# Vanvitelli-Robotics/uclv_qs_pushing_matlab

Measured on AMD Instinct MI355X. Metric: NMPC solves/sec at N=20, batch=65 536; max |u0−u0_ref|, higher is better.
Workload: dtype f64

## Files before the change

### uclv_qs_pushing_matlab_amd/csrc/qsp_capi.hip

```cpp
#include <hip/hip_runtime.h>

#include <cmath>
#include <cstdlib>
#include <cstdio>
#include <cstring>
#include <string>
#include <vector>

#include "../../include/qsp_nmpc.h"
#include "qsp_kernels.h"

using namespace qsp;

static thread_local std::string g_err;

static int fail(int code, const std::string& msg) {
    g_err = msg;
    return code;
}

#define HIPCHK(expr)                                                                                  \
    do {                                                                                              \
        hipError_t e_ = (expr);                                                                       \
        if (e_ != hipSuccess) return fail(QSP_ERR_HIP, std::string(#expr) + ": " + hipGetErrorString(e_)); \
    } while (0)

struct DevBuf {
    void* p = nullptr;
    size_t n = 0;
    hipError_t ensure(size_t bytes) {
        if (bytes <= n) return hipSuccess;
        if (p) (void)hipFree(p);
        p = nullptr;
        n = 0;
        hipError_t e = hipMalloc(&p, bytes);
        if (e == hipSuccess) n = bytes;
        return e;
    }
    void release() {
        if (p) (void)hipFree(p);
        p = nullptr;
        n = 0;
    }
    template <class T>
    T* as() const { return static_cast<T*>(p); }
};

struct qsp_solver {
    qsp_options o;
    SolveParams p;
    int S = 1;
    hipStream_t stream = nullptr;
    hipEvent_t ev0 = nullptr, ev1 = nullptr;
    int n_shapes = 0;
    DevBuf shapes, shape_id, x0, yref, yref_e, X, U, PI, Xo, Uo, PIo, u0, status, sqp_iter, qp_iter, qp_capped, qp_stalled, cost;
    DevBuf warm_valid, traj, index_time;
    int32_t D = 0;
    DevBuf ubc, ubp, cl_x, cl_xsim, cl_amp;
    DevBuf wX, wU, wx0, wlin, wnlp, wdone, wres, wqp, wperm, wnit, whist;
    DevBuf scratch[12];
    DevBuf ro[12];
    bool solved = false;
    int32_t T = 0;
    bool have_traj = false;
    bool traj_per_lane = false;
    float last_ms = 0.0f;
    bool last_controller = false;
    bool poison = false;
    std::vector<hipEvent_t> kev;
    int kev_used = 0;
    std::vector<int> kev_solves;
    std::vector<int> kev_split;
    bool auto_timing = false;
    SqpStreams split;
    int parts_req = 0;
    int fused_req = -1;
    bool nopack = false;
    bool mfw = true;
    int cus = 256;
};

static const SqpStreams* sqp_split(qsp_solver* s) {
    s->split.parts = s->parts_req > 0 ? s->parts_req : sqp_parts_auto(s->o.batch, s->o.N, s->S, s->cus);
    const bool can_fuse = s->o.nlp_mode == QSP_NLP_SQP_RTI_FIXED && (s->S == 1 || s->S == 2);
    s->split.fused = !can_fuse ? 0
                   : s->fused_req >= 0 ? s->fused_req
                   : (s->split.parts == 1 && sqp_fused_auto(s->o.batch, s->o.N, s->S, s->o.nlp_mode, s->cus));
    if (s->split.fused) s->split.parts = 1;
    return &s->split;
}

static hipEvent_t* take_kernel_events(qsp_solver* s) {
    const int per = 2 * s->o.sqp_iters + 3;
    if (s->auto_timing) {
        s->kev_used = 0;
        s->kev_solves.clear();
        s->kev_split.clear();
    }
    if (s->kev.empty() || s->kev_used + per > (int)s->kev.size()) return nullptr;
    s->kev_solves.push_back(s->kev_used);
    s->kev_split.push_back((sqp_split(s)->parts > 1 || s->split.fused) ? 1 : 0);
    hipEvent_t* e = s->kev.data() + s->kev_used;
    s->kev_used += per;
    return e;
}

static int kernel_times_of(qsp_solver* s, double* ms, int32_t* launches);

static void fill_params(qsp_solver* s) {
    SolveParams& p = s->p;
    p.N = s->o.N;
    p.nlp_mode = s->o.nlp_mode;
// ... 48 lines not shown
    for (int i = 0; i < nv; ++i) { xy[2 * i] = v[(size_t)i * nprop]; xy[2 * i + 1] = v[(size_t)i * nprop + 1]; }
    return QSP_OK;
}

static int h2d(qsp_solver* s, DevBuf& b, const void* src, size_t bytes) {
    HIPCHK(hipSetDevice(s->o.device));
    HIPCHK(hipMemcpyAsync(b.p, src, bytes, hipMemcpyHostToDevice, s->stream));
    HIPCHK(hipStreamSynchronize(s->stream));
    return QSP_OK;
}
static int d2h(qsp_solver* s, void* dst, const DevBuf& b, size_t bytes) {
    HIPCHK(hipSetDevice(s->o.device));
    HIPCHK(hipMemcpyAsync(dst, b.p, bytes, hipMemcpyDeviceToHost, s->stream));
    HIPCHK(hipStreamSynchronize(s->stream));
    return QSP_OK;
}

static SolveArgs make_args(qsp_solver* s) {
    SolveArgs a;
    std::memset(&a, 0, sizeof a);
    a.p = s->p;
    a.B = s->o.batch;
    a.shapes = s->shapes.as<ShapeDev>();
    a.n_shapes = s->n_shapes;
    a.shape_id = s->shape_id.as<int32_t>();
    a.x0 = s->x0.as<double>();
    a.yref = s->yref.as<double>();
    a.yref_e = s->yref_e.as<double>();
    a.X_in = s->X.as<double>();
    a.U_in = s->U.as<double>();
    a.u0 = s->u0.as<double>();
    a.X_out = s->Xo.as<double>();
    a.U_out = s->Uo.as<double>();
    a.PI_out = s->PIo.as<double>();
    s->last_controller = false;
    a.status = s->status.as<int32_t>();
    a.sqp_iter = s->sqp_iter.as<int32_t>();
    a.qp_iter = s->qp_iter.as<int32_t>();
    a.qp_capped = s->qp_capped.as<int32_t>();
    a.qp_stalled = s->qp_stalled.as<int32_t>();
    a.cost = s->cost.as<double>();
    a.wX = s->wX.as<double>();
    a.wU = s->wU.as<double>();
    a.wx0 = s->wx0.as<double>();
    a.wlin = s->wlin.as<double>();
    a.wnlp = s->wnlp.as<double>();
    a.wdone = s->wdone.as<int32_t>();
    a.wres = s->wres.as<double>();
    a.wqp = s->wqp.as<double>();
    a.wperm = s->nopack ? nullptr : s->wperm.as<int32_t>();
    if (s->poison) a.flags |= QSP_FLAG_POISON;
    a.wnit = s->wnit.as<int32_t>();
    a.whist = s->whist.as<int32_t>();
    a.PI_in = s->PI.as<double>();
    return a;
}

static int run_timed(qsp_solver* s, const SolveArgs& a) {
    HIPCHK(hipEventRecord(s->ev0, s->stream));
    HIPCHK(launch_sqp(a, s->S, s->stream, take_kernel_events(s), sqp_split(s)));
    HIPCHK(hipEventRecord(s->ev1, s->stream));
    HIPCHK(hipEventSynchronize(s->ev1));
    HIPCHK(hipEventElapsedTime(&s->last_ms, s->ev0, s->ev1));
    s->solved = true;
    return QSP_OK;
}

template <class T>
static int stage_in(qsp_solver* s, DevBuf& b, const T* src, size_t count) {
    HIPCHK(b.ensure(count * sizeof(T)));
    HIPCHK(hipMemcpyAsync(b.p, src, count * sizeof(T), hipMemcpyHostToDevice, s->stream));
    return QSP_OK;
}
template <class T>
static int stage_out(qsp_solver* s, T* dst, DevBuf& b, size_t count) {
    HIPCHK(hipMemcpyAsync(dst, b.p, count * sizeof(T), hipMemcpyDeviceToHost, s->stream));
    return QSP_OK;
}

static int check_ids(qsp_solver* s, int32_t n, const int32_t* ids) {
    if (s->n_shapes < 1) return fail(QSP_ERR_STATE, "no shapes set");
    for (int i = 0; i < n; ++i)
        if (ids[i] < 0 || ids[i] >= s->n_shapes) return fail(QSP_ERR_ARG, "shape id out of range");
    return QSP_OK;
}

__global__ void stage_yref_kernel(const double* traj, int T, int per_lane, const int32_t* index_time, int offset,
                                  int D, int B, int N, double* yref, double* yref_e) {
    const int i = blockIdx.x * blockDim.x + threadIdx.x;
    if (i >= B) return;
    if (per_lane) traj += (size_t)i * T * 6;
    for (int k = 0; k < N; ++k) {
        int idx = index_time[i] + offset + k;
        if (idx > T + D) idx = T + D;
        if (idx < 1) idx = 1;
        double* out = yref + ((size_t)i * N + k) * 6;
        if (idx <= D) {
            for (int c = 0; c < 5; ++c) out[c] = 0.0;
            out[5] = traj[5];
        } else {
            for (int c = 0; c < 6; ++c) out[c] = traj[(size_t)(idx - D - 1) * 6 + c];
        }
    }
    for (int c = 0; c < 4; ++c) yref_e[(size_t)i * 4 + c] = yref[((size_t)i * N + N - 1) * 6 + c];
}

// ... 87 lines not shown
        hipDeviceProp_t prop;
        if (hipGetDeviceProperties(&prop, o->device) == hipSuccess && prop.multiProcessorCount > 0)
            s->cus = prop.multiProcessorCount;
    }
    fill_params(s);
    const double W[6] = {1.0, 1.0, 1e-3, 0.0, 1e-3, 1e-3};
    const double We[4] = {2e5, 2e5, 20.0, 0.0};
    const double lh[3] = {-0.06, 0.0, -0.05}, uh[3] = {0.011, 0.03, 0.05};
    std::memcpy(s->p.W, W, sizeof W);
    std::memcpy(s->p.We, We, sizeof We);
    std::memcpy(s->p.lh, lh, sizeof lh);
    std::memcpy(s->p.uh, uh, sizeof uh);
    s->p.cp = CtrlParams{1.0, 0.0, 3.0, 0.0, 0.05};
    hipError_t e = hipStreamCreateWithFlags(&s->stream, hipStreamNonBlocking);
    if (e == hipSuccess) e = hipEventCreate(&s->ev0);
    if (e == hipSuccess) e = hipEventCreate(&s->ev1);
    if (e == hipSuccess) e = hipEventCreateWithFlags(&s->split.fork, hipEventDisableTiming);
    for (int q = 0; q < SQP_MAX_PARTS - 1; ++q) {
        if (e == hipSuccess) e = hipStreamCreateWithFlags(&s->split.aux[q], hipStreamNonBlocking);
        if (e == hipSuccess) e = hipEventCreateWithFlags(&s->split.join[q], hipEventDisableTiming);
    }
    const size_t B = o->batch, N = o->N;
    auto al = [&](DevBuf& b, size_t bytes) { if (e == hipSuccess) e = b.ensure(bytes); };
    al(s->shape_id, B * 4);
    al(s->x0, B * 4 * 8);
    al(s->yref, B * N * 6 * 8);
    al(s->yref_e, B * 4 * 8);
    al(s->X, B * (N + 1) * 4 * 8);
    al(s->U, B * N * 2 * 8);
    al(s->PI, B * N * 4 * 8);
    al(s->Xo, B * (N + 1) * 4 * 8);
    al(s->Uo, B * N * 2 * 8);
    al(s->PIo, B * N * 4 * 8);
    al(s->u0, B * 2 * 8);
    al(s->status, B * 4);
    al(s->sqp_iter, B * 4);
    al(s->qp_iter, B * 4);
    al(s->qp_capped, B * 4);
    al(s->qp_stalled, B * 4);
    al(s->cost, B * 8);
    al(s->warm_valid, B);
    al(s->wX, B * (N + 1) * 4 * 8);
    al(s->wU, B * N * 2 * 8);
    al(s->wx0, B * 4 * 8);
    al(s->wperm, B * 4);
    al(s->wnit, B * 4);
    al(s->whist, SQP_MAX_PARTS * 4 * 1024 * 4);
    al(s->wdone, B * 4);
    if (o->nlp_mode == QSP_NLP_SQP_MERIT) {
        al(s->wlin, B * (N + 1) * 24 * 8);
        al(s->wnlp, B * (N + 1) * 20 * 8);
        al(s->wqp, B * (N + 1) * 16 * 8);
        al(s->wres, B * 4 * 8);
    }
    if (e == hipSuccess) e = hipMemsetAsync(s->shape_id.p, 0, B * 4, s->stream);
    if (e == hipSuccess) e = hipMemsetAsync(s->warm_valid.p, 0, B, s->stream);
    if (e == hipSuccess) e = hipMemsetAsync(s->X.p, 0, B * (N + 1) * 4 * 8, s->stream);
    if (e == hipSuccess) e = hipMemsetAsync(s->U.p, 0, B * N * 2 * 8, s->stream);
    if (e == hipSuccess) e = hipMemsetAsync(s->PI.p, 0, B * N * 4 * 8, s->stream);
    if (const char* fl = std::getenv("QSP_FUSED_LOOP")) s->fused_req = (fl[0] == '1') ? 1 : (fl[0] == '0' ? 0 : -1);
    if (const char* pk = std::getenv("QSP_PACKING")) s->nopack = pk[0] == '0';
    if (const char* mw = std::getenv("QSP_MFMA_WALK")) s->mfw = mw[0] != '0';
    s->p.mfma_walk = s->mfw ? 1 : 0;
    mfw_prepare(s->p);
    const char* pz = std::getenv("QSP_DEBUG_POISON");
    s->poison = pz && pz[0] == '1';
    if (s->poison) {
        DevBuf* ws[] = {&s->wX, &s->wU, &s->wx0, &s->wlin, &s->wnlp, &s->wdone, &s->wres, &s->wqp, &s->wperm, &s->wnit,
                        &s->X, &s->U, &s->PI, &s->Xo, &s->Uo, &s->PIo, &s->u0, &s->cost, &s->yref, &s->yref_e};
        for (DevBuf* b : ws)
            if (e == hipSuccess && b->p) e = hipMemsetAsync(b->p, 0xff, b->n, s->stream);
        if (e == hipSuccess) e = hipMemsetAsync(s->X.p, 0, B * (N + 1) * 4 * 8, s->stream);
        if (e == hipSuccess) e = hipMemsetAsync(s->U.p, 0, B * N * 2 * 8, s->stream);
        if (e == hipSuccess) e = hipMemsetAsync(s->PI.p, 0, B * N * 4 * 8, s->stream);
    }
    if (e == hipSuccess && s->wres.p) e = hipMemsetAsync(s->wres.p, 0, B * 4 * 8, s->stream);
    if (e == hipSuccess) e = hipStreamSynchronize(s->stream);
    if (e != hipSuccess) {
        std::string m = std::string("qsp_create: ") + hipGetErrorString(e);
        qsp_destroy(s);
        return fail(QSP_ERR_HIP, m);
    }
    *out = s;
    return QSP_OK;
}

int qsp_destroy(qsp_solver* s) {
    if (!s) return QSP_OK;
    (void)hipSetDevice(s->o.device);
    DevBuf* bufs[] = {&s->ubc, &s->ubp, &s->cl_x, &s->cl_xsim, &s->cl_amp,
                      &s->shapes, &s->shape_id, &s->x0, &s->yref, &s->yref_e, &s->X, &s->U, &s->PI, &s->Xo,
                      &s->Uo, &s->PIo, &s->u0, &s->status, &s->sqp_iter, &s->qp_iter, &s->qp_capped, &s->qp_stalled, &s->cost,
                      &s->warm_valid,
                      &s->traj, &s->index_time, &s->wX, &s->wU, &s->wx0, &s->wlin, &s->wnlp, &s->wdone, &s->wres, &s->wqp, &s->wperm, &s->wnit,
                      &s->whist};
    for (DevBuf* b : bufs) b->release();
    for (auto& b : s->scratch) b.release();
    for (auto& b : s->ro) b.release();
    for (hipEvent_t e : s->kev) (void)hipEventDestroy(e);
    if (s->ev0) (void)hipEventDestroy(s->ev0);
    if (s->ev1) (void)hipEventDestroy(s->ev1);
    if (s->split.fork) (void)hipEventDestroy(s->split.fork);
    for (int q = 0; q < SQP_MAX_PARTS - 1; ++q) {
        if (s->split.join[q]) (void)hipEventDestroy(s->split.join[q]);
        if (s->split.aux[q]) (void)hipStreamDestroy(s->split.aux[q]);
    }
    if (s->stream) (void)hipStreamDestroy(s->stream);
    delete s;
    return QSP_OK;
}

int qsp_get_layout(const qsp_solver* s, int32_t* S, int32_t* L) {
    if (!s) return fail(QSP_ERR_ARG, "qsp_get_layout: null handle");
    if (S) *S = s->S;
    if (L) *L = lanes_per_instance(s->o.N, s->S);
    return QSP_OK;
}

int qsp_get_factor_walk(const qsp_solver* s, int32_t* walk) {
    if (!s || !walk) return fail(QSP_ERR_ARG, "qsp_get_factor_walk: null argument");
    *walk = factor_walk_kind(s->p, s->S);
    return QSP_OK;
}

int qsp_shape_from_ply(const char* path, int32_t flip, double mu_sg, double mu_sp, double mass, double tau_max,
                       qsp_shape* out) {
    if (!path || !out) return fail(QSP_ERR_ARG, "qsp_shape_from_ply: null argument");
    std::vector<float> P;
    int r = read_ply_xy(path, P);
    if (r != QSP_OK) return r;
    const int n0 = (int)(P.size() / 2);
    if (n0 + 1 > QSP_MAX_CTRL) return fail(QSP_ERR_ARG, "qsp_shape_from_ply: too many points");
    std::vector<float> xs(P);
    const float inf = INFINITY;
    int ind = 0;
    for (int i = 1; i < n0; ++i) if (xs[2 * i] < xs[2 * ind]) ind = i;
    float tx = xs[2 * ind], ty = xs[2 * ind + 1];
    xs[2 * ind] = xs[2 * ind + 1] = inf;
    std::vector<double> srt((size_t)(n0 + 1) * 2);
    srt[0] = tx; srt[1] = ty;
    for (int i = 1; i < n0; ++i) {
        int best = -1;
        float bd = 0.0f;
        for (int q = 0; q < n0; ++q) {
            const float dx = xs[2 * q] - tx, dy = xs[2 * q + 1] - ty;
            const float d = std::sqrt(dx * dx + dy * dy);
            if (best < 0 || d < bd) { best = q; bd = d; }
        }
// ... 909 lines not shown
```

### uclv_qs_pushing_matlab_amd/csrc/qsp_kernels.h

```cpp
#pragma once
#include <hip/hip_runtime.h>
#include <stdint.h>

#include "qsp_layout.h"
#include "qsp_types.h"

#define QSP_FLAG_CONTROLLER 1u
#define QSP_FLAG_SHIFT 2u
#define QSP_FLAG_POISON 4u

namespace qsp {

struct SolveArgs {
    SolveParams p;
    int32_t B;
    int32_t i0, nI;
    uint32_t flags;
    const ShapeDev* shapes;
    int32_t n_shapes;
    const int32_t* shape_id;
    const double* x0;
    const double* yref;
    const double* yref_e;
    const double* X_in;
    const double* U_in;
    uint8_t* warm_valid;
    const double* PI_in;
    double* u0;
    double* X_out;
    double* U_out;
    double* PI_out;
    int32_t* status;
    int32_t* sqp_iter;
    int32_t* qp_iter;
    int32_t* qp_capped;
    int32_t* qp_stalled;
    double* cost;
    double* wX;
    double* wU;
    double* wx0;
    double* wlin;
    double* wnlp;
    int32_t* wdone;
    double* wres;
    double* wqp;
    int32_t* wperm;
    int32_t* wnit;
    int32_t* whist;
    double* qp_dx;
    double* qp_du;
    double* qp_lam;
};

__device__ __forceinline__ int shape_clamp(int id, int n_shapes) { return id < 0 ? 0 : (id >= n_shapes ? n_shapes - 1 : id); }
__device__ __forceinline__ const ShapeDev& shape_clamped(const ShapeDev* shapes, int n_shapes, const int32_t* sid, int i) {
    return shapes[shape_clamp(sid ? sid[i] : 0, n_shapes)];
}

int factor_walk_kind(const SolveParams& p, int S);
void mfw_prepare(SolveParams& p);
constexpr int SQP_MAX_PARTS = 2;
struct SqpStreams {
    hipStream_t aux[SQP_MAX_PARTS - 1] = {};
    hipEvent_t fork = nullptr, join[SQP_MAX_PARTS - 1] = {};
    int parts = 1;
    int fused = 0;
};
hipError_t launch_sqp(const SolveArgs& a, int S, hipStream_t stream, hipEvent_t* ev = nullptr,
                      const SqpStreams* split = nullptr);
int sqp_parts_auto(int B, int N, int S, int cus);
int sqp_fused_auto(int B, int N, int S, int nlp_mode, int cus);
hipError_t launch_qp(const SolveArgs& a, int S, hipStream_t stream);
struct ClosedLoopArgs {
    const ShapeDev* shapes;
    int32_t n_shapes;
    const int32_t* sid;
    int32_t B, n_steps;
    double Ts;
    double* x;
    double* xs;
    const double* noise;
    int32_t dist_step;
    const double* dist_amp;
    int32_t D, Dp;
    double* ubc;
    double* ubp;
    const double* u0;
    const int32_t* status;
    double* Xtraj;
    double* Xsim;
    double* Utraj;
    int32_t* Straj;
};
hipError_t launch_closed_loop_pre(const ClosedLoopArgs& a, int t, hipStream_t stream);
hipError_t launch_plant(const ClosedLoopArgs& a, int t, hipStream_t stream);
hipError_t launch_delay_sim(const ClosedLoopArgs& a, hipStream_t stream);
hipError_t launch_reproject(const ShapeDev* shapes, int n_shapes, const int32_t* sid, int n, const double* px,
                            const double* py, const double* s0, double* s, hipStream_t stream);
hipError_t launch_straight_lines(int B, int T, const double* x0, const double* xf, double t0, double tf, double Ts,
                                 int auto_angle, double* traj, hipStream_t stream);
hipError_t launch_spline(const ShapeDev* shapes, const int32_t* sid, int n, const double* s, double* C, double* D,
// ... 38 lines not shown
```

### uclv_qs_pushing_matlab_amd/csrc/qsp_solver.hip

```cpp
#include <hip/hip_runtime.h>
#include <stdint.h>

#include <atomic>
#include <type_traits>

#include "../../include/qsp_nmpc.h"
#include "qsp_layout.h"
#include "qsp_math.hpp"
#include "qsp_kernels.h"

#ifndef QSP_MIN_WAVES
#define QSP_MIN_WAVES 1
#endif

namespace qsp {

#ifdef QSP_SEGSTAMP
#ifndef QSP_SEGMASK
#define QSP_SEGMASK 0xffffffffu
#endif
__device__ unsigned long long g_seg[32];
__device__ __forceinline__ unsigned long long seg_now() { return __builtin_amdgcn_s_memtime(); }
__device__ __forceinline__ void seg_add(int i, unsigned long long t0) {
    if (!((QSP_SEGMASK >> i) & 1u)) return;
// ... 1195 lines not shown
                }
            }
        }
#pragma unroll
        for (int i = 0; i < 4; ++i) dx[i] = wave_from_prev(dx[i]);
    }
}

__device__ __forceinline__ void adjoint_step(const SolveParams& p, const double a[6], const double dx[4],
                                             const double g[6], double dlam_s, double pi[4]) {
    double np[4];
    np[0] = qfma(p.tau * p.W[0], dx[0], g[0]) + pi[0];
    np[1] = qfma(p.tau * p.W[1], dx[1], g[1]) + pi[1];
    np[2] = qfma(p.tau * p.W[2], dx[2], g[2]) + (qfma(a[2], pi[1], a[0] * pi[0]) + pi[2]);
    np[3] = qfma(p.tau * p.W[3], dx[3], g[3]) + qfma(a[5], pi[3], qfma(a[4], pi[2], qfma(a[3], pi[1], a[1] * pi[0])));
    np[3] += dlam_s;
#pragma unroll
    for (int i = 0; i < 4; ++i) pi[i] = np[i];
}

template <int S>
__device__ __forceinline__ void qp_adjoint_store(const Ctx& c, const SolveParams& p, const Stage<S>& st,
                                                 double* PI, bool write, bool shift) {
    double pi[4] = {0, 0, 0, 0};
    for (int j = c.L - 1; j >= 0; --j) {
        if (c.lig == j) {
#pragma unroll
            for (int ls = S - 1; ls >= 0; --ls) {
                const int k = j * S + ls;
                if (k == c.N) {
#pragma unroll
                    for (int i = 0; i < 4; ++i) pi[i] = qfma(p.We[i], st.dxs(ls, i), st.g[ls][i]);
                } else if (k < c.N) {
                    if (write && (!shift || k >= 1)) {
#pragma unroll
                        for (int i = 0; i < 4; ++i) PI[(size_t)(shift ? k - 1 : k) * 4 + i] = pi[i];
                    }
                    if (write && shift && k == c.N - 1) {
#pragma unroll
                        for (int i = 0; i < 4; ++i) PI[(size_t)k * 4 + i] = pi[i];
                    }
                    if (k >= 1) {
                        const double dxk[4] = {st.dxs(ls, 0), st.dxs(ls, 1), st.dxs(ls, 2), st.dxs(ls, 3)};
                        adjoint_step(p, st.a[ls], dxk, st.g[ls], st.lm(ls, 1) - st.lm(ls, 0), pi);
                    }
                }
            }
        }
#pragma unroll
        for (int i = 0; i < 4; ++i) pi[i] = wave_from_next(pi[i]);
    }
}

enum LinField : int { L_A = 0, L_B = 6, L_BB = 14, L_G = 18, L_COUNT = 24 };

__device__ __forceinline__ const ShapeDev& shape_of(const SolveArgs& A, int i) {
    const int id = A.shape_id ? A.shape_id[i] : 0;
    return A.shapes[shape_clamp(id, A.n_shapes)];
}

enum NlpField : int { W_PI = 0, W_LAM = 4, W_NU = 10, W_ETA = 14, W_COUNT = 20 };

__device__ __forceinline__ void nlp_init(const SolveArgs& A, int i, bool use_pi) {
    const int N = A.p.N;
    const size_t tot = (size_t)A.B * (N + 1);
    for (int k = 0; k <= N; ++k) {
        const size_t si = (size_t)i * (N + 1) + k;
        for (int q = 0; q < 4; ++q)
            A.wnlp[(W_PI + q) * tot + si] = (use_pi && A.PI_in && k < N) ? A.PI_in[((size_t)i * N + k) * 4 + q] : 0.0;
        for (int q = W_LAM; q < W_COUNT; ++q) A.wnlp[q * tot + si] = 0.0;
    }
    A.wdone[i] = 0;
    if (A.wres)
        for (int q = 0; q < 4; ++q) A.wres[(size_t)i * 4 + q] = 0.0;
}

__device__ __forceinline__ void s0_feasible(const SolveArgs& A, int i, double s0) {
    const SolveParams& p = A.p;
    if (p.s0_bound && A.wdone && !(s0 >= p.lh[0] && s0 <= p.uh[0])) {
        A.wdone[i] = 3;
        A.sqp_iter[i] = 0;
    }
}

__global__ void prologue_kernel(SolveArgs A) {
    const int i = blockIdx.x * blockDim.x + threadIdx.x;
    if (i >= A.B) return;
    const SolveParams& p = A.p;
    const int N = p.N;
    const ShapeDev& sh = shape_of(A, i);
    double x0[4];
    for (int c = 0; c < 4; ++c) x0[c] = A.x0[(size_t)i * 4 + c];
    double* X = A.wX + (size_t)i * (N + 1) * 4;
    double* U = A.wU + (size_t)i * N * 2;
    A.qp_iter[i] = 0;
    if (A.qp_capped) A.qp_capped[i] = 0;
    if (A.qp_stalled) A.qp_stalled[i] = 0;
    if (A.wdone) A.wdone[i] = 0;
    if (A.wnit) A.wnit[i] = 0;
    if (!(A.flags & QSP_FLAG_CONTROLLER)) {
        for (int q = 0; q < (N + 1) * 4; ++q) X[q] = A.X_in[(size_t)i * (N + 1) * 4 + q];
        for (int q = 0; q < N * 2; ++q) U[q] = A.U_in[(size_t)i * N * 2 + q];
        for (int c = 0; c < 4; ++c) A.wx0[(size_t)i * 4 + c] = x0[c];
        if (p.nlp_mode == 1) nlp_init(A, i, true);
        s0_feasible(A, i, x0[3]);
        return;
    }
    x0[3] = qfma(-sh.b, (x0[3] < 0.0) ? 1.0 : 0.0, mat_mod(x0[3], sh.b));
    for (int c = 0; c < 4; ++c) A.wx0[(size_t)i * 4 + c] = x0[c];
    const bool cold = (A.warm_valid == nullptr || A.warm_valid[i] == 0);
    if (p.nlp_mode == 1) nlp_init(A, i, !cold);
    for (int k = 0; k < N; ++k) {
        U[2 * k] = cold ? p.cp.u_n_lb : A.U_in[((size_t)i * N + k) * 2];
        U[2 * k + 1] = cold ? 0.0 : A.U_in[((size_t)i * N + k) * 2 + 1];
    }
    double xc[4] = {x0[0], x0[1], x0[2], x0[3]};
    for (int k = 0; k <= N; ++k) {
        for (int c = 0; c < 4; ++c) X[4 * k + c] = xc[c];
        if (k == N) break;
        const double vb = v_bound(sh, p.cp, xc[3]);
        const double ut_old = U[2 * k + 1];
        if (fabs(ut_old) > vb) {
            const double sgn = ut_old > 0.0 ? 1.0 : -1.0;
            U[2 * k + 1] = sgn * vb;
            U[2 * k] = U[2 * k + 1] * U[2 * k] / ut_old;
        }
        DynOut d;
        dynamics<false>(sh, xc[2], xc[3], U[2 * k], U[2 * k + 1], d);
        for (int c = 0; c < 4; ++c) xc[c] = qfma(p.Ts, d.f[c], xc[c]);
    }
    s0_feasible(A, i, x0[3]);
}

__device__ __forceinline__ void qp_adjoint_lane(const Ctx& c, const SolveParams& p, const Stage<1>& st,
                                                double piq[4]) {
    double pi[4] = {0, 0, 0, 0};
#pragma unroll
    for (int i = 0; i < 4; ++i) piq[i] = 0.0;
    for (int j = c.L - 1; j >= 0; --j) {
        if (c.lig == j) {
            if (j == c.N) {
#pragma unroll
                for (int i = 0; i < 4; ++i) pi[i] = qfma(p.We[i], st.dxs(0, i), st.g[0][i]);
            } else {
#pragma unroll
                for (int i = 0; i < 4; ++i) piq[i] = pi[i];
                if (j >= 1) {
                    const double dxk[4] = {st.dxs(0, 0), st.dxs(0, 1), st.dxs(0, 2), st.dxs(0, 3)};
                    adjoint_step(p, st.a[0], dxk, st.g[0], st.lm(0, 1) - st.lm(0, 0), pi);
                }
            }
        }
// ... 262 lines not shown
            A.wdone[iv] = 1;
            A.sqp_iter[iv] = it;
        }
    }
    int exit;
    SEG_NEXT(10, t_k);
    const int nit = qp_ipm<S, ALT>(c, p, st, dx0, exit, skip);
    SEG_NEXT(11, t_k);
    qp_rollout<S>(c, st, dx0);
    const bool failed = qp_outcome<S>(A, c, st, iv, it, exit, skip);
    if (A.wnit && c.real && c.lig == 0) {
        const int old = A.wnit[iv];
        const int rec = (MERIT || !(skip || failed)) ? pack_record(old, nit) : old;
        A.wnit[iv] = rec;
        if (A.whist) atomicAdd(&A.whist[(it & 1) * PACK_KEYS_MAX + pack_key(rec, pack_maxkey(p.qp_iters))], 1);
    }
    if constexpr (MERIT) {
        double piq[4];
        qp_adjoint_lane(c, p, st, piq);
        if (c.real && !skip && !failed) {
            const size_t si = (size_t)iv * (N + 1) + c.lig;
            double* w = A.wqp + si;
#pragma unroll
            for (int q = 0; q < 4; ++q) w[(Q_DX + q) * tot] = st.dxs(0, q);
#pragma unroll
            for (int q = 0; q < 2; ++q) w[(Q_DU + q) * tot] = c.lig < N ? st.du(0, q) : 0.0;
#pragma unroll
            for (int q = 0; q < 4; ++q) w[(Q_PI + q) * tot] = piq[q];
#pragma unroll
            for (int q = 0; q < 6; ++q) w[(Q_LAM + q) * tot] = c.lig < N ? st.lm(0, q) : 0.0;
        }
        if (c.real && c.lig == 0) A.qp_iter[iv] += nit;
        return;
    }
    const bool last = it + 1 >= p.sqp_iters;
    if (A.qp_dx) {
        if (last) qp_adjoint_store<S>(c, p, st, A.PI_out + (size_t)iv * N * 4, c.real, false);
        if (!c.real) return;
#pragma unroll
        for (int ls = 0; ls < S; ++ls) {
            const int k = kof<S>(c, ls);
            if (k <= N)
                for (int q = 0; q < 4; ++q) A.qp_dx[((size_t)iv * (N + 1) + k) * 4 + q] = st.dxs(ls, q);
            if (k < N) {
                for (int q = 0; q < 2; ++q) A.qp_du[((size_t)iv * N + k) * 2 + q] = st.du(ls, q);
                for (int q = 0; q < 6; ++q) A.qp_lam[((size_t)iv * N + k) * 6 + q] = st.lm(ls, q);
            }
            if (k == 0) A.qp_iter[iv] = nit;
            if (k == 0 && A.qp_capped)
                A.qp_capped[iv] = exit == QP_EXIT_CONV ? 0 : (exit == QP_EXIT_CAP ? 2 : (exit == QP_EXIT_STALL ? 4 : 5));
        }
        return;
    }
    qp_adjoint_store<S>(c, p, st, A.PI_out + (size_t)iv * N * 4, c.real && !skip && !failed,
                        (A.flags & QSP_FLAG_SHIFT) != 0);
    if (!c.real || skip || failed) return;
    iterate_update<S>(A, c, st, iv, nit, X, U);
    SEG_ADD(12, t_k);
}

template <int S, bool ALT = false>
__global__ void __launch_bounds__(BLOCK, QSP_MIN_WAVES) sqp_loop_kernel(SolveArgs A) {
    extern __shared__ double smem[];
    const SolveParams& p = A.p;
    const int N = p.N;
    if (A.flags & QSP_FLAG_POISON) poison_lds<S>(smem + threadIdx.x);
    bool stopped = false;
    for (int it = 0; it < p.sqp_iters; ++it) {
        if (it > 0) __syncthreads();
        if (it > 0 && (A.flags & QSP_FLAG_POISON)) poison_lds<S>(smem + threadIdx.x);
        int lane = threadIdx.x & 63;
        asm volatile("" : "+v"(lane));
        const Ctx c = ctx_of<S>(lane, N, A.nI);
        const int iv = A.i0 + (c.real ? c.inst : A.nI - 1);
        double* X = A.wX + (size_t)iv * (N + 1) * 4;
        double* U = A.wU + (size_t)iv * N * 2;
        if (it == 0) stopped = A.wdone[iv] != 0;
        Stage<S> st;
        st.lds = smem + threadIdx.x;
        const bool lin_live = c.real && !stopped;
#pragma unroll
        for (int ls = 0; ls < S; ++ls) {
            const int k = kof<S>(c, ls);
            const int kc = k <= N ? k : N;
            const int ku = k < N ? k : N - 1;
            if (kc < N && lin_live) {
                const double xk[4] = {X[4 * kc], X[4 * kc + 1], X[4 * kc + 2], X[4 * kc + 3]};
                const double uk[2] = {U[2 * kc], U[2 * kc + 1]};
                Lin Ln;
                rk4<true>(shape_of(A, iv), p.Ts, xk, uk, Ln);
                const double* yr = A.yref + ((size_t)iv * N + kc) * 6;
#pragma unroll
                for (int q = 0; q < 6; ++q) st.a[ls][q] = Ln.a[q];
#pragma unroll
                for (int q = 0; q < 8; ++q) st.B[ls][q] = Ln.B[q];
#pragma unroll
                for (int q = 0; q < 4; ++q) st.bb[ls][q] = Ln.xn[q] - X[4 * (kc + 1) + q];
#pragma unroll
                for (int q = 0; q < 4; ++q) st.g[ls][q] = p.tau * p.W[q] * (xk[q] - yr[q]);
#pragma unroll
                for (int q = 0; q < 2; ++q) st.g[ls][4 + q] = p.tau * p.W[4 + q] * (uk[q] - yr[4 + q]);
            } else {
                const double* ye = A.yref_e + (size_t)iv * 4;
#pragma unroll
                for (int q = 0; q < 6; ++q) st.a[ls][q] = 0.0;
#pragma unroll
                for (int q = 0; q < 8; ++q) st.B[ls][q] = 0.0;
#pragma unroll
                for (int q = 0; q < 4; ++q) st.bb[ls][q] = 0.0;
#pragma unroll
                for (int q = 0; q < 4; ++q) st.g[ls][q] = p.We[q] * (X[4 * N + q] - ye[q]);
                st.g[ls][4] = 0.0;
                st.g[ls][5] = 0.0;
            }
            load_bounded<S>(st, ls, kc, ku, X, U);
        }
        double dx0[4];
#pragma unroll
        for (int q = 0; q < 4; ++q) dx0[q] = A.wx0[(size_t)iv * 4 + q] - X[q];
        const bool skip = stopped || !c.real;
        int exit;
        const int nit = qp_ipm<S, ALT>(c, p, st, dx0, exit, skip);
        qp_rollout<S>(c, st, dx0);
        const bool failed = qp_outcome<S>(A, c, st, iv, it, exit, skip);
        qp_adjoint_store<S>(c, p, st, A.PI_out + (size_t)iv * N * 4, c.real && !skip && !failed,
                            (A.flags & QSP_FLAG_SHIFT) != 0);
        if (c.real && !skip && !failed) iterate_update<S>(A, c, st, iv, nit, X, U);
        stopped = stopped || failed;
    }
}

__global__ void __launch_bounds__(256) sort_by_iters_kernel(int i0, int B, int maxkey, const int32_t* nit,
                                                            int32_t* perm, int32_t* whist, int q) {
    constexpr int KPT = PACK_KEYS_MAX / 256;
    __shared__ int pre[PACK_KEYS_MAX], lcount[PACK_KEYS_MAX], part[256];
    const int tid = threadIdx.x;
    const int nkeys = (maxkey + 1) * (maxkey + 1);
    const int32_t* hist = whist + q * PACK_KEYS_MAX;
    int32_t* run = whist + (2 + q) * PACK_KEYS_MAX;
    int h[KPT], sum = 0;
#pragma unroll
    for (int r = 0; r < KPT; ++r) {
        const int k = tid * KPT + r;
        h[r] = k < nkeys ? hist[k] : 0;
        sum += h[r];
        lcount[k] = 0;
    }
    part[tid] = sum;
    __syncthreads();
    for (int off = 1; off < 256; off <<= 1) {
        const int v = tid >= off ? part[tid - off] : 0;
        __syncthreads();
        part[tid] += v;
        __syncthreads();
    }
    int acc = part[tid] - sum;
#pragma unroll
    for (int r = 0; r < KPT; ++r) {
        pre[tid * KPT + r] = acc;
        acc += h[r];
    }
    __syncthreads();
    const int i = blockIdx.x * blockDim.x + tid;
    int key = 0, pos = 0;
    if (i < B) {
        key = pack_key(nit[i0 + i], maxkey);
        pos = atomicAdd(&lcount[key], 1);
    }
    __syncthreads();
#pragma unroll
    for (int r = 0; r < KPT; ++r) {
        const int k = tid * KPT + r;
        if (lcount[k] > 0) pre[k] += atomicAdd(&run[k], lcount[k]);
    }
    __syncthreads();
    if (i < B) perm[i0 + pre[key] + pos] = i0 + i;
    if (blockIdx.x == 0) {
#pragma unroll
        for (int r = 0; r < KPT; ++r) {
            whist[(1 - q) * PACK_KEYS_MAX + tid * KPT + r] = 0;
// ... 125 lines not shown
#pragma unroll
        for (int q = 0; q < 4; ++q) nw[(W_NU + q) * tot] = NUk[q];
#pragma unroll
        for (int q = 0; q < 6; ++q) nw[(W_ETA + q) * tot] = ETAk[q];
    }
}

__global__ void epilogue_kernel(SolveArgs A) {
    const int i = blockIdx.x * blockDim.x + threadIdx.x;
    if (i >= A.B) return;
    const SolveParams& p = A.p;
    const int N = p.N;
    const double* X = A.wX + (size_t)i * (N + 1) * 4;
    const double* U = A.wU + (size_t)i * N * 2;
    const double* yref = A.yref + (size_t)i * N * 6;
    const double* ye = A.yref_e + (size_t)i * 4;
    bool bad = false;
    double cost = 0.0;
    for (int k = 0; k < N; ++k) {
        double s = 0.0;
        for (int q = 0; q < 4; ++q) { const double r = X[4 * k + q] - yref[6 * k + q]; s = qfma(p.W[q] * r, r, s); bad |= !isfinite(X[4 * k + q]); }
        for (int q = 0; q < 2; ++q) { const double r = U[2 * k + q] - yref[6 * k + 4 + q]; s = qfma(p.W[4 + q] * r, r, s); bad |= !isfinite(U[2 * k + q]); }
        cost = qfma(0.5 * p.tau, s, cost);
    }
    double s = 0.0;
    for (int q = 0; q < 4; ++q) { const double r = X[4 * N + q] - ye[q]; s = qfma(p.We[q] * r, r, s); bad |= !isfinite(X[4 * N + q]); }
    cost = qfma(0.5, s, cost);
    A.cost[i] = cost;
    const int fr = A.wdone ? A.wdone[i] : 0;
    if (fr == 3 || fr == 4) A.status[i] = QSP_STATUS_QP_FAIL;
    else if (p.nlp_mode == 1) A.status[i] = (bad || fr == 2) ? 1 : (fr == 1 ? 0 : 2);
    else A.status[i] = (bad || fr == 2) ? 1 : 0;
    if (fr == 0) A.sqp_iter[i] = p.sqp_iters;
    A.u0[(size_t)i * 2] = U[0];
    A.u0[(size_t)i * 2 + 1] = U[1];
    const int sh = (A.flags & QSP_FLAG_SHIFT) ? 1 : 0;
    double* Xo = A.X_out + (size_t)i * (N + 1) * 4;
    double* Uo = A.U_out + (size_t)i * N * 2;
    for (int k = 0; k <= N; ++k) {
        const int src = (k + sh <= N) ? k + sh : N;
        for (int q = 0; q < 4; ++q) Xo[4 * k + q] = X[4 * src + q];
    }
    for (int k = 0; k < N; ++k) {
        const int src = (k + sh < N) ? k + sh : N - 1;
        for (int q = 0; q < 2; ++q) Uo[2 * k + q] = U[2 * src + q];
    }
    if (p.nlp_mode == 1) {
        const size_t tot = (size_t)A.B * (N + 1);
        double* Po = A.PI_out + (size_t)i * N * 4;
        for (int k = 0; k < N; ++k) {
            const int src = (k + sh < N) ? k + sh : N - 1;
            for (int q = 0; q < 4; ++q) Po[4 * k + q] = A.wnlp[(W_PI + q) * tot + (size_t)i * (N + 1) + src];
        }
    }
    if (A.warm_valid && (A.flags & QSP_FLAG_CONTROLLER)) A.warm_valid[i] = 1;
}


__device__ __forceinline__ double contact_phi(const ShapeDev& sh, double s, double px, double py) {
    SplineEval e;
    spline_eval(sh, mat_mod(s, sh.b), e);
    const double ex = e.C[0] - px, ey = e.C[1] - py;
    return qfma(ey, ey, ex * ex);
}

__device__ double reproject_contact(const ShapeDev& sh, double px, double py, double s0) {
    double s = s0, phi = contact_phi(sh, s, px, py);
    for (int it = 0; it < 60; ++it) {
        SplineEval e;
        spline_eval(sh, mat_mod(s, sh.b), e);
        const double ex = e.C[0] - px, ey = e.C[1] - py;
        const double g = 2.0 * qfma(ey, e.D[1], ex * e.D[0]);
        const double h = 2.0 * qfma(ey, e.Dd[1], qfma(ex, e.Dd[0], qfma(e.D[1], e.D[1], e.D[0] * e.D[0])));
        if (fabs(g) < 1e-14) break;
        double step = h > 0.0 ? -g / h : (g > 0.0 ? -0.05 : 0.05) * sh.b;
        const double smax = 0.25 * sh.b;
        step = fmin(fmax(step, -smax), smax);
        bool ok = false;
        double sn = s, phin = phi;
        for (int k = 0; k < 60; ++k) {
            sn = s + step;
            phin = contact_phi(sh, sn, px, py);
            if (phin < phi) { ok = true; break; }
            step *= 0.5;
        }
        if (!ok) break;
        s = sn;
        phi = phin;
        if (fabs(step) < 1e-13 * sh.b) break;
    }
    return s;
}

__global__ void closed_loop_pre_kernel(ClosedLoopArgs a, int t) {
    const int i = blockIdx.x * blockDim.x + threadIdx.x;
    if (i >= a.B) return;
    const ShapeDev& sh = shape_clamped(a.shapes, a.n_shapes, a.sid, i);
    double x[4] = {a.x[(size_t)i * 4], a.x[(size_t)i * 4 + 1], a.x[(size_t)i * 4 + 2], a.x[(size_t)i * 4 + 3]};
    if (a.dist_step > 0 && t + 1 == a.dist_step) {
        const double amp = a.dist_amp ? a.dist_amp[i] : 0.0;
        x[1] += amp;
        SplineEval e;
        spline_eval(sh, mat_mod(x[3], sh.b), e);
        const double sn = reproject_contact(sh, -0.5 * sh.xwidth, e.C[1] - amp, 0.0);
        x[3] = qfma(-sh.b, sn < 0.0 ? 1.0 : 0.0, mat_mod(sn, sh.b));
    }
// ... 221 lines not shown

int sqp_fused_auto(int B, int N, int S, int nlp_mode, int cus) {
    const long waves = waves_for(B, N, S);
    return (nlp_mode == 0 && (S == 1 || S == 2) && waves <= 4L * cus) ? 1 : 0;
}

static hipError_t launch_qp_any(const SolveArgs& a, int S, int it, hipStream_t stream, bool lin) {
    return with_variant(a.p, S, [&](auto s, auto alt) {
        return lin ? launch_qp_waves<qp_step_kernel<s(), false, true, alt()>, s()>(a, stream, it)
                   : launch_qp_waves<qp_step_kernel<s(), false, false, alt()>, s()>(a, stream, it);
    });
}

#ifdef QSP_SEGSTAMP
extern "C" int qsp_debug_segments(unsigned long long* out, int reset) {
    if (hipMemcpyFromSymbol(out, HIP_SYMBOL(g_seg), sizeof(g_seg)) != hipSuccess) return -2;
    if (reset) {
        static const unsigned long long zero[32] = {};
        if (hipMemcpyToSymbol(HIP_SYMBOL(g_seg), zero, sizeof(zero)) != hipSuccess) return -2;
    }
    return 0;
}
#endif

static hipError_t launch_sqp_merit(const SolveArgs& a, int it, hipStream_t stream) {
    const hipError_t e = factor_alt(a.p, 1) ? launch_qp_waves<qp_step_kernel<1, true, true, true>, 1>(a, stream, it)
                                            : launch_qp_waves<qp_step_kernel<1, true, true, false>, 1>(a, stream, it);
    if (e != hipSuccess) return e;
    hipLaunchKernelGGL(merit_ls_kernel, dim3((unsigned)waves_for(a.nI, a.p.N, 1)), dim3(WAVE), 0, stream, a);
    return hipGetLastError();
}

int sqp_parts_auto(int B, int N, int S, int cus) {
    const long waves = waves_for(B, N, S);
    return waves >= 8L * cus ? 2 : 1;
}

template <class Mark>
static hipError_t sqp_iteration(const SolveArgs& as, int S, bool sorted, int it, hipStream_t stream, Mark&& mark) {
    hipError_t e = hipSuccess;
    if (sorted && it > 0) {
        hipLaunchKernelGGL(sort_by_iters_kernel, dim3((as.nI + 255) / 256), dim3(256), 0, stream, as.i0, as.nI,
                           pack_maxkey(as.p.qp_iters), as.wnit, as.wperm, as.whist, (it - 1) & 1);
        e = hipGetLastError();
    }
    if (e == hipSuccess) e = mark();
    if (e == hipSuccess)
        e = as.p.nlp_mode == 1 ? launch_sqp_merit(as, it, stream) : launch_qp_any(as, S, it, stream, true);
    if (e == hipSuccess) e = mark();
    return e;
}

hipError_t launch_sqp(const SolveArgs& a, int S, hipStream_t stream, hipEvent_t* ev, const SqpStreams* split) {
    const int G = instances_per_wave(a.p.N, S);
    int P = split ? split->parts : 1;
    if (P > SQP_MAX_PARTS) P = SQP_MAX_PARTS;
    const int wtot = (int)waves_for(a.B, a.p.N, S);
    if (P > wtot) P = wtot;
    for (int q = 1; q < P; ++q)
        if (!split->aux[q - 1] || !split->join[q - 1] || !split->fork) P = 1;
    const bool fused = split && split->fused && a.p.nlp_mode == 0 && a.wdone && (S == 1 || S == 2);
    if (fused) P = 1;
    const bool two = P > 1;
    const int K = a.p.sqp_iters;
    int ne = 0;
    auto mark = [&]() { return ev ? hipEventRecord(ev[ne++], stream) : hipSuccess; };
    auto nomark = []() { return hipSuccess; };
    const unsigned gb = (unsigned)((a.B + 127) / 128);
    hipError_t e = mark();
    if (e != hipSuccess) return e;
    hipLaunchKernelGGL(prologue_kernel, dim3(gb), dim3(128), 0, stream, a);
    e = hipGetLastError();
    const bool sorted = !fused && a.wperm && a.wnit && a.whist;
    SolveArgs as = a;
    as.i0 = 0;
    as.nI = a.B;
    if (!sorted) {
        as.whist = nullptr;
        as.wperm = nullptr;
    }
    if (e == hipSuccess && sorted) {
        hipLaunchKernelGGL(iota_kernel, dim3(gb), dim3(128), 0, stream, a.B, a.wperm);
        e = hipGetLastError();
        if (e == hipSuccess)
            e = hipMemsetAsync(a.whist, 0, P * 4 * PACK_KEYS_MAX * sizeof(int32_t), stream);
    }
    if (e == hipSuccess) e = mark();
    if (fused) {
        if (e == hipSuccess)
            e = with_variant(as.p, S, [&](auto s, auto alt) {
                return launch_qp_waves<sqp_loop_kernel<s(), alt()>, s()>(as, stream);
            });
        ne = 2 * K + 1;
        if (e == hipSuccess) e = mark();
    } else if (!two) {
        for (int it = 0; it < K && e == hipSuccess; ++it) e = sqp_iteration(as, S, sorted, it, stream, mark);
    } else {
        SolveArgs ap[SQP_MAX_PARTS];
        hipStream_t sp[SQP_MAX_PARTS];
        for (int q = 0; q < P; ++q) {
            const int w0 = (int)((long)wtot * q / P), w1 = (int)((long)wtot * (q + 1) / P);
            ap[q] = as;
            ap[q].i0 = w0 * G;
            ap[q].nI = (q + 1 < P ? w1 * G : a.B) - w0 * G;
            if (sorted) ap[q].whist = a.whist + q * 4 * PACK_KEYS_MAX;
            sp[q] = q == 0 ? stream : split->aux[q - 1];
// ... 49 lines not shown
```

Before: 616,300.

## Defer adjoint backward recursion to epilogue using per-stage recorded coefficients

Instead of running the costate backward recursion inside every SQP/QP iteration, each iteration now writes a compact per-stage record (gradient terms, dynamics Jacobian entries and multiplier difference) to a workspace buffer. The epilogue then runs the recursion once from the last valid record to fill PI_out, handling the shift option. This removes a serial backward pass, and likely a cross-lane dependency, from the hot QP loop. In exchange it adds 11 doubles per stage of global-memory writes per iteration and a new workspace allocation.

```diff
diff --git a/uclv_qs_pushing_matlab_amd/csrc/qsp_capi.hip b/uclv_qs_pushing_matlab_amd/csrc/qsp_capi.hip
--- a/uclv_qs_pushing_matlab_amd/csrc/qsp_capi.hip
+++ b/uclv_qs_pushing_matlab_amd/csrc/qsp_capi.hip
@@ -57,7 +57,7 @@
     DevBuf warm_valid, traj, index_time;
     int32_t D = 0;
     DevBuf ubc, ubp, cl_x, cl_xsim, cl_amp;
-    DevBuf wX, wU, wx0, wlin, wnlp, wdone, wres, wqp, wperm, wnit, whist;
+    DevBuf wX, wU, wx0, wlin, wnlp, wdone, wres, wqp, wperm, wnit, whist, wadj, wadjv;
     DevBuf scratch[12];
     DevBuf ro[12];
     bool solved = false;
@@ -212,6 +212,8 @@
     if (s->poison) a.flags |= QSP_FLAG_POISON;
     a.wnit = s->wnit.as<int32_t>();
     a.whist = s->whist.as<int32_t>();
+    a.wadj = s->wadj.as<double>();
+    a.wadjv = s->wadjv.as<int32_t>();
     a.PI_in = s->PI.as<double>();
     return a;
 }
@@ -405,6 +407,9 @@
         al(s->wnlp, B * (N + 1) * 20 * 8);
         al(s->wqp, B * (N + 1) * 16 * 8);
         al(s->wres, B * 4 * 8);
+    } else {
+        al(s->wadj, B * N * 11 * 8);
+        al(s->wadjv, B * 4);
     }
     if (e == hipSuccess) e = hipMemsetAsync(s->shape_id.p, 0, B * 4, s->stream);
     if (e == hipSuccess) e = hipMemsetAsync(s->warm_valid.p, 0, B, s->stream);
@@ -420,7 +425,7 @@
     s->poison = pz && pz[0] == '1';
     if (s->poison) {
         DevBuf* ws[] = {&s->wX, &s->wU, &s->wx0, &s->wlin, &s->wnlp, &s->wdone, &s->wres, &s->wqp, &s->wperm, &s->wnit,
-                        &s->X, &s->U, &s->PI, &s->Xo, &s->Uo, &s->PIo, &s->u0, &s->cost, &s->yref, &s->yref_e};
+                        &s->wadj, &s->wadjv, &s->X, &s->U, &s->PI, &s->Xo, &s->Uo, &s->PIo, &s->u0, &s->cost, &s->yref, &s->yref_e};
         for (DevBuf* b : ws)
             if (e == hipSuccess && b->p) e = hipMemsetAsync(b->p, 0xff, b->n, s->stream);
         if (e == hipSuccess) e = hipMemsetAsync(s->X.p, 0, B * (N + 1) * 4 * 8, s->stream);
@@ -446,7 +451,7 @@
                       &s->Uo, &s->PIo, &s->u0, &s->status, &s->sqp_iter, &s->qp_iter, &s->qp_capped, &s->qp_stalled, &s->cost,
                       &s->warm_valid,
                       &s->traj, &s->index_time, &s->wX, &s->wU, &s->wx0, &s->wlin, &s->wnlp, &s->wdone, &s->wres, &s->wqp, &s->wperm, &s->wnit,
-                      &s->whist};
+                      &s->whist, &s->wadj, &s->wadjv};
     for (DevBuf* b : bufs) b->release();
     for (auto& b : s->scratch) b.release();
     for (auto& b : s->ro) b.release();
diff --git a/uclv_qs_pushing_matlab_amd/csrc/qsp_kernels.h b/uclv_qs_pushing_matlab_amd/csrc/qsp_kernels.h
--- a/uclv_qs_pushing_matlab_amd/csrc/qsp_kernels.h
+++ b/uclv_qs_pushing_matlab_amd/csrc/qsp_kernels.h
@@ -47,6 +47,8 @@
     int32_t* wperm;
     int32_t* wnit;
     int32_t* whist;
+    double* wadj;
+    int32_t* wadjv;
     double* qp_dx;
     double* qp_du;
     double* qp_lam;
diff --git a/uclv_qs_pushing_matlab_amd/csrc/qsp_solver.hip b/uclv_qs_pushing_matlab_amd/csrc/qsp_solver.hip
--- a/uclv_qs_pushing_matlab_amd/csrc/qsp_solver.hip
+++ b/uclv_qs_pushing_matlab_amd/csrc/qsp_solver.hip
@@ -1271,6 +1271,55 @@
     }
 }
 
+constexpr int ADJ_REC = 11;
+
+template <int S>
+__device__ __forceinline__ void qp_adjoint_record(const Ctx& c, const SolveParams& p, const Stage<S>& st, double* rec) {
+#pragma unroll
+    for (int ls = 0; ls < S; ++ls) {
+        const int k = kof<S>(c, ls);
+        if (k < 1 || k > c.N) continue;
+        double* r = rec + (size_t)(k - 1) * ADJ_REC;
+        if (k == c.N) {
+#pragma unroll
+            for (int i = 0; i < 4; ++i) r[i] = qfma(p.We[i], st.dxs(ls, i), st.g[ls][i]);
+        } else {
+#pragma unroll
+            for (int i = 0; i < 4; ++i) r[i] = qfma(p.tau * p.W[i], st.dxs(ls, i), st.g[ls][i]);
+#pragma unroll
+            for (int i = 0; i < 6; ++i) r[4 + i] = st.a[ls][i];
+            r[10] = st.lm(ls, 1) - st.lm(ls, 0);
+        }
+    }
+}
+
+__device__ __forceinline__ void adjoint_from_record(int N, const double* rec, double* PI, bool shift) {
+    double pi[4];
+#pragma unroll
+    for (int i = 0; i < 4; ++i) pi[i] = rec[(size_t)(N - 1) * ADJ_REC + i];
+    for (int k = N - 1; k >= 0; --k) {
+        if (!shift || k >= 1) {
+#pragma unroll
+            for (int i = 0; i < 4; ++i) PI[(size_t)(shift ? k - 1 : k) * 4 + i] = pi[i];
+        }
+        if (shift && k == N - 1) {
+#pragma unroll
+            for (int i = 0; i < 4; ++i) PI[(size_t)k * 4 + i] = pi[i];
+        }
+        if (k >= 1) {
+            const double* r = rec + (size_t)(k - 1) * ADJ_REC;
+            double np[4];
+            np[0] = r[0] + pi[0];
+            np[1] = r[1] + pi[1];
+            np[2] = r[2] + (qfma(r[6], pi[1], r[4] * pi[0]) + pi[2]);
+            np[3] = r[3] + qfma(r[9], pi[3], qfma(r[8], pi[2], qfma(r[7], pi[1], r[5] * pi[0])));
+            np[3] += r[10];
+#pragma unroll
+            for (int i = 0; i < 4; ++i) pi[i] = np[i];
+        }
+    }
+}
+
 enum LinField : int { L_A = 0, L_B = 6, L_BB = 14, L_G = 18, L_COUNT = 24 };
 
 __device__ __forceinline__ const ShapeDev& shape_of(const SolveArgs& A, int i) {
@@ -1317,6 +1366,7 @@
     if (A.qp_stalled) A.qp_stalled[i] = 0;
     if (A.wdone) A.wdone[i] = 0;
     if (A.wnit) A.wnit[i] = 0;
+    if (A.wadjv) A.wadjv[i] = 0;
     if (!(A.flags & QSP_FLAG_CONTROLLER)) {
         for (int q = 0; q < (N + 1) * 4; ++q) X[q] = A.X_in[(size_t)i * (N + 1) * 4 + q];
         for (int q = 0; q < N * 2; ++q) U[q] = A.U_in[(size_t)i * N * 2 + q];
@@ -1685,9 +1735,11 @@
         }
         return;
     }
-    qp_adjoint_store<S>(c, p, st, A.PI_out + (size_t)iv * N * 4, c.real && !skip && !failed,
-                        (A.flags & QSP_FLAG_SHIFT) != 0);
     if (!c.real || skip || failed) return;
+    SEG_NEXT(12, t_k);
+    qp_adjoint_record<S>(c, p, st, A.wadj + (size_t)iv * N * ADJ_REC);
+    if (c.lig == 0) A.wadjv[iv] = 1;
+    SEG_NEXT(16, t_k);
     iterate_update<S>(A, c, st, iv, nit, X, U);
     SEG_ADD(12, t_k);
 }
@@ -1756,9 +1808,11 @@
         const int nit = qp_ipm<S, ALT>(c, p, st, dx0, exit, skip);
         qp_rollout<S>(c, st, dx0);
         const bool failed = qp_outcome<S>(A, c, st, iv, it, exit, skip);
-        qp_adjoint_store<S>(c, p, st, A.PI_out + (size_t)iv * N * 4, c.real && !skip && !failed,
-                            (A.flags & QSP_FLAG_SHIFT) != 0);
-        if (c.real && !skip && !failed) iterate_update<S>(A, c, st, iv, nit, X, U);
+        if (c.real && !skip && !failed) {
+            qp_adjoint_record<S>(c, p, st, A.wadj + (size_t)iv * N * ADJ_REC);
+            if (c.lig == 0) A.wadjv[iv] = 1;
+            iterate_update<S>(A, c, st, iv, nit, X, U);
+        }
         stopped = stopped || failed;
     }
 }
@@ -1990,6 +2044,9 @@
             const int src = (k + sh < N) ? k + sh : N - 1;
             for (int q = 0; q < 4; ++q) Po[4 * k + q] = A.wnlp[(W_PI + q) * tot + (size_t)i * (N + 1) + src];
         }
+    }
+    if (p.nlp_mode == 0 && A.wadjv && A.wadjv[i] != 0) {
+        adjoint_from_record(N, A.wadj + (size_t)i * N * ADJ_REC, A.PI_out + (size_t)i * N * 4, sh != 0);
     }
     if (A.warm_valid && (A.flags & QSP_FLAG_CONTROLLER)) A.warm_valid[i] = 1;
 }
@@ -2317,6 +2374,7 @@
 }
 
 hipError_t launch_sqp(const SolveArgs& a, int S, hipStream_t stream, hipEvent_t* ev, const SqpStreams* split) {
+    if (a.p.nlp_mode == 0 && (!a.wadj || !a.wadjv)) return hipErrorInvalidValue;
     const int G = instances_per_wave(a.p.N, S);
     int P = split ? split->parts : 1;
     if (P > SQP_MAX_PARTS) P = SQP_MAX_PARTS;
```

Measured after the change: 626,800, median of 6. 1.02x the previous value.
